# tjysdsg/speech-recognition

Hardware: AMD Instinct MI355X
Metric: frame-state loglik/s + utterances/s Viterbi decode (higher is better)
Workload: dtype f64; 1 GPU; configs[1]: 10-digit HMM, 5 states/digit, 8-mix GMM, 39-dim, 10000 utterances/GPU (999364 frames on rank 0), isolated-word decode; states=50, mixtures=8, dim=39, parallelism=utterance-sharded x1, batches_in_flight=2, process_group=single

## Files before the change

### speech-recognition_amd/csrc/gh_internal.h

```cpp
#pragma once
#include <hip/hip_runtime.h>
#include <stdint.h>
#include <stdarg.h>
#include <stdio.h>
#include <string>
#include <vector>
#include "../../include/gmmhmm.h"

void gh_set_error(const char* fmt, ...);

#define GH_HIP(call)                                                                     \
    do {                                                                                 \
        hipError_t e_ = (call);                                                          \
        if (e_ != hipSuccess) {                                                          \
            gh_set_error("%s:%d %s -> %s", __FILE__, __LINE__, #call, hipGetErrorString(e_)); \
            return (e_ == hipErrorOutOfMemory) ? GH_ERR_NOMEM : GH_ERR_HIP;              \
        }                                                                                \
    } while (0)

#define GH_REQUIRE(cond, ...)                 \
    do {                                      \
        if (!(cond)) {                        \
            gh_set_error(__VA_ARGS__);        \
            return GH_ERR_INVALID;            \
        }                                     \
    } while (0)

#define GH_LEAN_NARROW_ARCS 3

#define GH_LSE_SCALE64 184.66496523378731614
#define GH_LSE_SCALE32 1.4426950408889634074
#define GH_LSE_OFF64 (-1e300)
#define GH_LSE_OFF32 (-1e30f)

struct gh_ctx {
    int device;
    hipStream_t stream;
    int n_cu;
    void* scratch;
    size_t scratch_bytes;
    int* d_flag;
    void* pinned;
    size_t pinned_bytes;
    double* d_fp64_tables;
    int compat;
    int last_fused = 0;
    int last_chunks;
    size_t budget_cache = 0;
    int budget_age = 0;
    void* fit_arena = nullptr;
    size_t fit_arena_bytes = 0;
    void* fit_pin = nullptr;
    void* fit_act = nullptr;
    size_t fit_act_bytes = 0;
};

int gh_scratch(gh_ctx* ctx, size_t bytes, void** out);
size_t gh_scratch_budget(gh_ctx* ctx, bool fresh = false);
int gh_pinned(gh_ctx* ctx, size_t bytes, void** out);

struct gh_gmm {
    gh_ctx* ctx;
    void* d_arena;
    int S, M, D, KP;
    std::vector<double> hA, hB, hC;
    bool host_stale = false;
    double *dA64, *dB64, *dC64;
    float *dA32, *dB32, *dC32;
    float* dCen32;
    double *dMean, *dIvar, *dLogc;
    int* dAnyPos = nullptr;
    int any_pos_host = -1;
    int M_pad, n_tiles;
    double *dApk64, *dCpk64;
    float *dApk32, *dCpk32;
    uint64_t serial = 0;
};
uint64_t gh_next_serial();

#define GH_FBCHAIN_MAX 16
struct gh_fbchain {
    int32_t n, pad;
    int32_t state[GH_FBCHAIN_MAX];
    double c0;
    double self_c[GH_FBCHAIN_MAX], next_c[GH_FBCHAIN_MAX], skip_c[GH_FBCHAIN_MAX];
};

struct gh_batch {
    gh_ctx* ctx;
    gh_dtype dtype;
    int D;
    int64_t N, U;
    void* feats;
    bool owns_feats;
    std::vector<int64_t> offsets;
    int64_t* d_offsets;
    int64_t max_T;
    bool any_T1 = false;
// ... 173 lines not shown
```

### speech-recognition_amd/csrc/gh_loglik_mfma.hip

```cpp
#include <type_traits>
#include "gh_internal.h"
#include "gh_wave.h"

namespace {

typedef double v4d __attribute__((ext_vector_type(4)));
typedef float v4f __attribute__((ext_vector_type(4)));

struct gh_loglik_blk { int64_t n0; int32_t nrows, t0, t1, pad; };

template <typename T> struct Acc;
template <> struct Acc<double> {
    typedef v4d type;
    static __device__ __forceinline__ v4d mfma(double a, double b, v4d c) {
        return __builtin_amdgcn_mfma_f64_16x16x4f64(a, b, c, 0, 0, 0);
    }
};
template <> struct Acc<float> {
    typedef v4f type;
    static __device__ __forceinline__ v4f mfma(float a, float b, v4f c) {
        return __builtin_amdgcn_mfma_f32_16x16x4f32(a, b, c, 0, 0, 0);
    }
};

struct Fp64Tables {
    double exp2[128];
    double inv[128];
    double nlog[128];
};

template <typename T> struct Dom;
template <> struct Dom<double> {
    static constexpr double inv_k = 1.0 / GH_LSE_SCALE64, off = GH_LSE_OFF64, off_test = GH_LSE_OFF64 * 0.1;
};
template <> struct Dom<float> {
    static constexpr float inv_k = (float)(1.0 / GH_LSE_SCALE32), off = GH_LSE_OFF32, off_test = GH_LSE_OFF32 * 0.1f;
};

struct LseK {
    double e3 = 2.6466421444330968834e-08;
    double l4 = -46.166241308446829036, l3 = 61.554988411262438714;
    double l2 = -92.332482616893658071, l1 = 184.66496523378731614;
    __device__ __forceinline__ void pin() {
        asm volatile("" : "+v"(e3), "+v"(l4), "+v"(l3), "+v"(l2), "+v"(l1));
    }
};

__device__ __forceinline__ double logs(double s, const double* __restrict__ tab, const LseK& k) {
    const double* __restrict__ inv = tab + 128;
    const double* __restrict__ nlog = tab + 256;
    const double m = __builtin_amdgcn_frexp_mant(s);
    const int e = __builtin_amdgcn_frexp_exp(s);
    const int j = (__double2hiint(m) >> 13) & 127;
    const double rho = fma(m, inv[j], -1.0);
    double p = fma(rho, 36.932993046757463228, k.l4);
    p = fma(p, rho, k.l3);
    p = fma(p, rho, k.l2);
    p = fma(p, rho, k.l1);
    return fma(p, rho, nlog[j]) + (double)(e << 7);
}
__device__ __forceinline__ float logs(float s, const double*, const LseK&) { return __builtin_amdgcn_logf(s); }

template <int W> __device__ __forceinline__ void swap_rows(unsigned v, unsigned& a, unsigned& b) {
    if (W == 16) {
        auto r = __builtin_amdgcn_permlane16_swap(v, v, false, false);
        a = r[0]; b = r[1];
    } else {
// ... 27 lines not shown
template <typename T> __device__ __forceinline__ T pair_max_split(T v0, T v1) { T a, b; pair_split(v0, v1, a, b); return vmax(a, b); }

template <typename T> __device__ __forceinline__ T nll_of(T mx, T sm, const double* tab, T inf_below, const LseK& k) {
    const T v = (mx + logs(sm, tab, k)) * -Dom<T>::inv_k;
    return (mx < inf_below) ? T(INFINITY) : v;
}

template <typename T, typename V> __device__ __forceinline__ T lane_max(const V& a) { return vmax(vmax(a[0], a[1]), vmax(a[2], a[3])); }
template <typename T, typename V> __device__ __forceinline__ T lane_terms(const V& a, T m, const double* tab, const LseK& k) {
    return (exp2s(a[0] - m, tab, k.e3) + exp2s(a[1] - m, tab, k.e3)) + (exp2s(a[2] - m, tab, k.e3) + exp2s(a[3] - m, tab, k.e3));
}
template <typename T, typename V>
__device__ __forceinline__ void tile_lse(const V& a, int width, T& mx, T& sm, const double* tab, const LseK& k) {
    T m = lane_max<T, V>(a);
    if (width >= 2) m = pair_max<T, 16>(m);
    if (width >= 4) m = pair_max<T, 32>(m);
    T e = lane_terms<T, V>(a, m, tab, k);
    if (width >= 2) e = pair_sum<T, 16>(e);
    if (width >= 4) e = pair_sum<T, 32>(e);
    mx = m;
    sm = e;
}

__device__ __forceinline__ float exp2s_fe(double y) { return __builtin_amdgcn_exp2f((float)y * 0.0078125f); }
template <int W> __device__ __forceinline__ float pair_sum_f(float v) { float a, b; pair_of<W>(v, a, b); return a + b; }
template <typename V>
__device__ __forceinline__ void tile_lse_fe(const V& a, int width, double& mx, float& sm) {
    double m = vmax(vmax(a[0], a[1]), vmax(a[2], a[3]));
    if (width >= 2) m = pair_max<double, 16>(m);
    if (width >= 4) m = pair_max<double, 32>(m);
    float e = (exp2s_fe(a[0] - m) + exp2s_fe(a[1] - m)) + (exp2s_fe(a[2] - m) + exp2s_fe(a[3] - m));
    if (width >= 2) e = pair_sum_f<16>(e);
    if (width >= 4) e = pair_sum_f<32>(e);
    mx = m;
    sm = e;
}
__device__ __forceinline__ double nll_of_fe(double mx, float sm, double inf_below) {
    const double v = (mx + (double)(128.0f * __builtin_amdgcn_logf(sm))) * -Dom<double>::inv_k;
    return (mx < inf_below) ? (double)INFINITY : v;
}

template <typename T> using global_ptr = const T __attribute__((address_space(1)))*;
template <typename T> __device__ __forceinline__ global_ptr<T> uniform_ptr(const T* p) {
    uint32_t lo = (uint32_t)reinterpret_cast<uintptr_t>(p), hi = (uint32_t)(reinterpret_cast<uintptr_t>(p) >> 32);
    asm("" : "+s"(lo), "+s"(hi));
    return (global_ptr<T>)reinterpret_cast<const T*>(((uintptr_t)hi << 32) | lo);
}

template <typename T, typename V, int MP, bool FE = false, bool CHK = true>
__device__ __forceinline__ void tile_epilogue(const V& acc0, const V& acc1, int t, int f, int q, int S, int RS,
                                              int chunk_s0, int tiles_per_state, T* lds, T* dummy,
                                              const double* tab, T (&run_mx)[2], T (&run_sm)[2], T inf_below, const LseK& k) {
    T* orow0 = lds + f * RS - chunk_s0;
    T* orow1 = orow0 + 16 * RS;
    if (MP == 1) {
        const int s = 16 * t + 4 * q;
#pragma unroll
        for (int c = 0; c < 2; ++c) {
            const V& acc = c ? acc1 : acc0;
            T* orow = c ? orow1 : orow0;
#pragma unroll
            for (int r = 0; r < 4; ++r)
                *((!CHK || s + r < S) ? orow + s + r : dummy) = (acc[r] < inf_below) ? T(INFINITY) : acc[r] * -Dom<T>::inv_k;
        }
    } else if (MP == 2) {
        const int s = 8 * t + 2 * q;
#pragma unroll
        for (int c = 0; c < 2; ++c) {
            const V& acc = c ? acc1 : acc0;
            T* orow = c ? orow1 : orow0;
#pragma unroll
            for (int h = 0; h < 2; ++h) {
                const T x0 = acc[2 * h], x1 = acc[2 * h + 1];
                const T m = vmax(x0, x1);
                const T e = exp2s(x0 - m, tab, k.e3) + exp2s(x1 - m, tab, k.e3);
                *((!CHK || s + h < S) ? orow + s + h : dummy) = nll_of<T>(m, e, tab, inf_below, k);
            }
        }
#ifdef GH_MF_NOEPI
    } else if (MP <= 16) {
        const int s = (16 / MP) * t + q / (MP / 4);
        *(((q & (MP / 4 - 1)) == 0 && (!CHK || s < S)) ? orow0 + s : dummy) = -((acc0[0] + acc0[1]) + (acc0[2] + acc0[3]));
        *(((q & (MP / 4 - 1)) == 0 && (!CHK || s < S)) ? orow1 + s : dummy) = -((acc1[0] + acc1[1]) + (acc1[2] + acc1[3]));
#endif
    } else if (FE && MP == 4) {
        if constexpr (FE) {
// ... 27 lines not shown
                const float e = exp2s_fe((d > 0.0) ? -d : d);
                const float rs = (float)run_sm[c];
                run_sm[c] = (double)((d > 0.0) ? fmaf(smf, e, rs) : fmaf(rs, e, smf));
                run_mx[c] = (d > 0.0) ? run_mx[c] : mx;
            }
            const bool odd = q & 1;
            const double v = nll_of_fe(odd ? run_mx[1] : run_mx[0], (float)(odd ? run_sm[1] : run_sm[0]), inf_below);
            *((last && q < 2) ? (odd ? orow1 : orow0) + s : dummy) = v;
#pragma unroll
            for (int c = 0; c < 2; ++c) {
                run_mx[c] = last ? Dom<T>::off : run_mx[c];
                run_sm[c] = last ? T(0) : run_sm[c];
            }
        }
    } else if (MP == 4) {
        T mx, sm;
        const int s = 4 * t + q;
        tile_lse<T, V>(acc0, 1, mx, sm, tab, k);
        *((!CHK || s < S) ? orow0 + s : dummy) = nll_of<T>(mx, sm, tab, inf_below, k);
        tile_lse<T, V>(acc1, 1, mx, sm, tab, k);
        *((!CHK || s < S) ? orow1 + s : dummy) = nll_of<T>(mx, sm, tab, inf_below, k);
    } else if (MP <= 16) {
        constexpr int width = MP / 4;
        T mxs = pair_max_split(lane_max<T, V>(acc0), lane_max<T, V>(acc1));
        if (width >= 4) mxs = pair_max<T, 32>(mxs);
        T mx0, mx1;
        pair_of<16>(mxs, mx0, mx1);
        T sm = pair_sum_split(lane_terms<T, V>(acc0, mx0, tab, k), lane_terms<T, V>(acc1, mx1, tab, k));
        if (width >= 4) sm = pair_sum<T, 32>(sm);
        const bool odd = q & 1;
        const int s = (16 / MP) * t + q / width;
        const T v = nll_of<T>(mxs, sm, tab, inf_below, k);
        *(((q & (width - 1)) < 2 && (!CHK || s < S)) ? (odd ? orow1 : orow0) + s : dummy) = v;
    } else {
        const bool last = (t + 1) % tiles_per_state == 0;
        const int s = t / tiles_per_state;
#pragma unroll
        for (int c = 0; c < 2; ++c) {
            T mx, sm;
            tile_lse<T, V>(c ? acc1 : acc0, 4, mx, sm, tab, k);
            const T d = run_mx[c] - mx;
            const T e = exp2s((d > T(0)) ? -d : d, tab, k.e3);
            run_sm[c] = (d > T(0)) ? fma(sm, e, run_sm[c]) : fma(run_sm[c], e, sm);
            run_mx[c] = (d > T(0)) ? run_mx[c] : mx;
        }
        const bool odd = q & 1;
        const T v = nll_of<T>(odd ? run_mx[1] : run_mx[0], odd ? run_sm[1] : run_sm[0], tab, inf_below, k);
        *((last && q < 2) ? (odd ? orow1 : orow0) + s : dummy) = v;
#pragma unroll
        for (int c = 0; c < 2; ++c) {
            run_mx[c] = last ? Dom<T>::off : run_mx[c];
            run_sm[c] = last ? T(0) : run_sm[c];
        }
    }
}

#ifndef GH_MF_SGB
#define GH_MF_SGB 0
#endif
template <typename T, int KS, int MP, bool MULTI, bool FE = false>
__global__ __launch_bounds__(64, (sizeof(T) == 4 ? 3 : 1)) void loglik_mfma_kernel(const T* __restrict__ X, int64_t N, int D,
                                                         const T* __restrict__ Apk, const T* __restrict__ Cpk,
                                                         int n_tiles, int S, int M_pad, int chunk_tiles,
                                                         const double* __restrict__ tables, int tab_off,
                                                         T* __restrict__ out, int bpw,
                                                         const gh_loglik_blk* __restrict__ blk_tab, int64_t n_blk,
                                                         const T* __restrict__ cen, T inf_below) {
    typedef typename Acc<T>::type V;
#ifndef GH_MF_RING32
#define GH_MF_RING32 2
#endif
#ifndef GH_MF_RING64
#define GH_MF_RING64 1
#endif
    constexpr int R = KS / (sizeof(T) == 4 ? GH_MF_RING32 : GH_MF_RING64);
    extern __shared__ __attribute__((aligned(16))) unsigned char smem_raw[];
    T* lds = reinterpret_cast<T*>(smem_raw);
    const int lane = threadIdx.x;
    const int f = lane & 15, q = lane >> 4;
    const int64_t n_blocks = (N + 31) / 32;
    int64_t n0 = (int64_t)blockIdx.x * (MULTI ? bpw : 1) * 32;
#ifdef GH_MF_TIMING
    long long tk[5], tw[2];
    tk[0] = clock64(); tw[0] = wall_clock64();
#endif
    int nrows = 0;
    const bool subset = MULTI && blk_tab != nullptr;
    const int64_t kb0 = (int64_t)blockIdx.x * (MULTI ? bpw : 1);
    int t_lo = subset ? blk_tab[kb0].t0 : 0, t_hi = n_tiles, nxt_t0 = 0;
    double* tab = reinterpret_cast<double*>(smem_raw + tab_off);
    if (sizeof(T) == 8 && MP != 1) {
        double tr[6];
#pragma unroll
        for (int it = 0; it < 6; ++it) tr[it] = tables[lane + 64 * it];
#pragma unroll
        for (int it = 0; it < 6; ++it) tab[lane + 64 * it] = tr[it];
    }
    auto stage_frames = [&]() {
        const int nelem = nrows * D;
        const T* src = X + n0 * D;
        T xr[KS];
#pragma unroll
        for (int it = 0; it < KS; ++it) {
            const int i = lane + 64 * it;
            xr[it] = (i < nelem) ? src[i] : T(0);
        }
#pragma unroll
        for (int it = 0; it < KS; ++it) {
            const int i = lane + 64 * it;
            if (i < nelem) lds[i] = xr[it];
        }
        __syncthreads();
    };
    constexpr int KQ = KS / 2;
    T b[2][KS];
    T cen_r[KQ];
#pragma unroll
    for (int j = 0; j < KQ; ++j) cen_r[j] = (sizeof(T) == 4 && cen) ? cen[4 * j + q] : T(0);
    auto build_b = [&]() {
#pragma unroll
        for (int c = 0; c < 2; ++c) {
            const int row = 16 * c + f;
#pragma unroll
            for (int j = 0; j < KQ; ++j) {
                const int d = 4 * j + q;
                T v = (row < nrows && d < D) ? lds[row * D + d] : T(0);
                if (sizeof(T) == 4) v = (row < nrows && d < D) ? v - cen_r[j] : T(0);
                b[c][j] = v * v;
                b[c][KQ + j] = v;
            }
        }
        __syncthreads();
    };

    const int tiles_per_state = (MP <= 16) ? 1 : M_pad / 16;
    const int SC = (MP <= 16) ? chunk_tiles * (16 / (MP <= 16 ? MP : 16)) : chunk_tiles / tiles_per_state;
    const int RS = (S <= SC) ? S : SC;
    T* dummy = lds + 32 * RS + lane;
    T run_mx[2] = {Dom<T>::off, Dom<T>::off}, run_sm[2] = {T(0), T(0)};
    LseK lse_k;
    if (sizeof(T) == 8 && !MULTI && !FE && MP != 1) lse_k.pin();
    int chunk_s0 = 0;
    int subset_cnt = 0;

    T ring[R];
#pragma unroll
    for (int j = 0; j < R; ++j) ring[j] = Apk[((int64_t)t_lo * KS + j) * 64 + lane];
    V c_a, c_b, p0, p1;
#pragma unroll
    for (int r = 0; r < 4; ++r) c_a[r] = Cpk[t_lo * 16 + 4 * q + r];

    auto mfma_tile = [&](int t, V& acc0, V& acc1, const V& c_use, V& c_load) {
        const int tn = (!MULTI || t + 1 < t_hi) ? t + 1 : nxt_t0;
        const global_ptr<T> cp = uniform_ptr(Cpk + (unsigned)(tn * 16));
#pragma unroll
        for (int r = 0; r < 4; ++r) c_load[r] = cp[4 * q + r];
        constexpr int WIN = 4096 / (64 * (int)sizeof(T)), NW = (KS + WIN - 1) / WIN;
        global_ptr<T> a_cur[NW], a_nxt[NW];
#pragma unroll
        for (int w = 0; w < NW; ++w) {
            a_cur[w] = uniform_ptr(Apk + (unsigned)(t * (KS * 64) + w * (WIN * 64)));
            a_nxt[w] = uniform_ptr(Apk + (unsigned)(tn * (KS * 64) + w * (WIN * 64)));
        }
#pragma unroll
// ... 46 lines not shown
            const gh_loglik_blk bd = blk_tab[k];
            n0 = bd.n0; nrows = bd.nrows; t_lo = bd.t0; t_hi = bd.t1;
            nxt_t0 = (ib + 1 < nb && k + 1 < n_blk) ? blk_tab[k + 1].t0 : bd.t0;
        } else {
            if (MULTI && n0 >= N) break;
            nrows = (int)((N - n0 < 32) ? (N - n0) : 32);
        }
        if (!(subset && ib > 0 && n0 == staged_n0)) {
#ifdef GH_MF_PRIO
            __builtin_amdgcn_s_setprio(3);
#endif
            stage_frames();
            build_b();
#ifdef GH_MF_PRIO
            __builtin_amdgcn_s_setprio(0);
#endif
            staged_n0 = n0;
        }
        chunk_s0 = (MP <= 16) ? t_lo * (16 / (MP <= 16 ? MP : 16)) : t_lo / tiles_per_state;
        if (subset) {
            const int s_end = (MP <= 16) ? t_hi * (16 / (MP <= 16 ? MP : 16)) : t_hi / tiles_per_state;
            subset_cnt = ((s_end < S) ? s_end : S) - chunk_s0;
        }
#ifdef GH_MF_TIMING
        tk[1] = clock64();
        tk[2] = tk[1];
#endif
        auto epi = [&](const V& e0, const V& e1, int t, auto chk) {
            tile_epilogue<T, V, MP, FE, decltype(chk)::value>(e0, e1, t, f, q, S, RS, chunk_s0, tiles_per_state, lds, dummy, tab, run_mx, run_sm, inf_below, lse_k);
#pragma unroll
            for (int i = 0; i < (GH_MF_SGB ? 2 * KS : 0); ++i) {
                __builtin_amdgcn_sched_group_barrier(0x008, 1, 0);
                __builtin_amdgcn_sched_group_barrier(0x002, sizeof(T) == 8 ? 5 : 3, 0);
            }
            if (!subset && (t + 1) % chunk_tiles == 0 && t + 1 < n_tiles) flush();
        };
        V r0, r1;
        const int tb = MULTI ? t_lo : 0, te = MULTI ? t_hi : n_tiles;
        mfma_tile(tb, p0, p1, c_a, c_b);
        if (sizeof(T) == 8) {
            int t = tb + 1;
            for (; t + 1 < te; t += 2) {
                mfma_tile(t, r0, r1, c_b, c_a);
                epi(p0, p1, t - 1, std::false_type());
                mfma_tile(t + 1, p0, p1, c_a, c_b);
                epi(r0, r1, t, std::false_type());
            }
            if (t < te) {
                mfma_tile(t, r0, r1, c_b, c_a);
                epi(p0, p1, t - 1, std::false_type());
                epi(r0, r1, t, std::true_type());
            } else {
                epi(p0, p1, te - 1, std::true_type());
                if (MULTI) c_a = c_b;
            }
        } else {
            for (int t = tb + 1; t < te; ++t) {
                mfma_tile(t, r0, r1, c_b, c_a);
// ... 54 lines not shown
            runs.push_back({t0, t1});
        }
        std::sort(runs.begin(), runs.end());
        size_t w = 0;
        for (size_t i = 0; i < runs.size(); ++i) {
            if (w > 0 && runs[i].first <= runs[w - 1].second) runs[w - 1].second = std::max(runs[w - 1].second, runs[i].second);
            else runs[w++] = runs[i];
        }
        runs.resize(w);
        for (const auto& tr : runs) {
            const int t0 = tr.first, t1 = tr.second;
            const int span = (M_pad <= 16) ? (t1 - t0) * (16 / M_pad) : (t1 - t0) / (M_pad / 16);
            if (span > SC) return 1;
            max_tiles = std::max(max_tiles, t1 - t0);
        }
        for (int64_t f = b->offsets[u]; f < b->offsets[u + 1]; f += 32)
            for (const auto& tr : runs)
                tabv.push_back(gh_loglik_blk{f, (int32_t)std::min<int64_t>(32, b->offsets[u + 1] - f), tr.first, tr.second, 0});
    }
    *max_tiles_out = max_tiles;
    return GH_OK;
}

template <typename T>
int launch_mfma_t(gh_ctx* ctx, const gh_gmm* g, gh_batch* b, const T* Apk, const T* Cpk, const int32_t* st_lo,
                  const int32_t* st_hi, const T* cen, const int64_t* rng_off, const gh_loglik_plan* plan) {
    const int64_t N = b->N;
    if (N == 0) return GH_OK;
    const int KS = g->KP / 2;
    const int M_pad = g->M_pad, n_tiles = g->n_tiles, S = g->S;
    int chunk_tiles, SC;
    chunk_shape(g, &chunk_tiles, &SC);
    size_t lds = ((size_t)32 * std::max(std::min(SC, S), g->D) + 64) * sizeof(T);
    lds = (lds + 15) & ~size_t(15);
    const int tab_off = (int)lds;
    if (sizeof(T) == 8 && M_pad != 1) lds += 384 * sizeof(double);
    const double* tables = ctx->d_fp64_tables;
    const T inf_below = (ctx->compat & 1) ? (T)(-745.1332191019412 * (sizeof(T) == 8 ? GH_LSE_SCALE64 : GH_LSE_SCALE32)) : Dom<T>::off_test;
    gh_loglik_blk* d_blk = nullptr;
    int64_t n_blk = 0;
    int max_tiles = n_tiles;
    if (plan) {
        d_blk = static_cast<gh_loglik_blk*>(plan->d_blk);
        n_blk = plan->n_blk;
        max_tiles = plan->max_tiles;
        if (n_blk == 0) return GH_OK;
    } else if (st_lo) {
        std::vector<gh_loglik_blk> tabv;
        int rc = build_blk_table(g, b, SC, st_lo, st_hi, rng_off, tabv, &max_tiles);
        if (rc) return rc;
        n_blk = (int64_t)tabv.size();
        if (n_blk == 0) return GH_OK;
        void* base;
        rc = gh_scratch(ctx, tabv.size() * sizeof(gh_loglik_blk), &base);
        if (rc) return rc;
        d_blk = static_cast<gh_loglik_blk*>(base);
        GH_HIP(hipMemcpyAsync(d_blk, tabv.data(), tabv.size() * sizeof(gh_loglik_blk), hipMemcpyHostToDevice, ctx->stream));
        GH_HIP(hipStreamSynchronize(ctx->stream));
    }
    const bool subset = plan || st_lo;
    const int64_t n_blocks = subset ? n_blk : (N + 31) / 32;
    const int per_block = std::max(1, max_tiles * KS * 2);
    int bpw = (int)std::max<int64_t>(1, std::min<int64_t>(8, (512 + per_block - 1) / per_block));
    if (const char* e = getenv("GMMHMM_LOGLIK_BPW")) bpw = std::max(1, std::min(16, atoi(e)));
    if (subset) bpw = std::max(bpw, 2);
    const unsigned grid = (unsigned)((n_blocks + bpw - 1) / bpw);
    const T* X = static_cast<const T*>(b->feats);
    T* out = static_cast<T*>(b->nll);
    const bool fe = sizeof(T) == 8 && (ctx->compat & 2) && M_pad >= 4;
#define GH_MF_LAUNCH(ks, mp)                                                                                             \
    do {                                                                                                                 \
        if (fe && sizeof(T) == 8 && mp >= 4) {                                                                           \
            if (bpw > 1)                                                                                                 \
                hipLaunchKernelGGL((loglik_mfma_kernel<T, ks, mp, true, (sizeof(T) == 8 && mp >= 4)>), dim3(grid), dim3(64), lds, ctx->stream, X, N, g->D, \
                                   Apk, Cpk, n_tiles, S, M_pad, chunk_tiles, tables, tab_off, out, bpw, d_blk, n_blk, cen, inf_below); \
            else                                                                                                         \
                hipLaunchKernelGGL((loglik_mfma_kernel<T, ks, mp, false, (sizeof(T) == 8 && mp >= 4)>), dim3(grid), dim3(64), lds, ctx->stream, X, N, g->D, \
                                   Apk, Cpk, n_tiles, S, M_pad, chunk_tiles, tables, tab_off, out, bpw, d_blk, n_blk, cen, inf_below); \
        } else if (bpw > 1)                                                                                                     \
            hipLaunchKernelGGL((loglik_mfma_kernel<T, ks, mp, true>), dim3(grid), dim3(64), lds, ctx->stream, X, N, g->D, \
                               Apk, Cpk, n_tiles, S, M_pad, chunk_tiles, tables, tab_off, out, bpw, d_blk, n_blk, cen, inf_below); \
        else                                                                                                             \
            hipLaunchKernelGGL((loglik_mfma_kernel<T, ks, mp, false>), dim3(grid), dim3(64), lds, ctx->stream, X, N, g->D, \
                               Apk, Cpk, n_tiles, S, M_pad, chunk_tiles, tables, tab_off, out, bpw, d_blk, n_blk, cen, inf_below); \
    } while (0)
#define GH_MF_CASE(ks)                                   \
    case ks:                                             \
        switch (M_pad) {                                 \
            case 1: GH_MF_LAUNCH(ks, 1); break;          \
            case 2: GH_MF_LAUNCH(ks, 2); break;          \
            case 4: GH_MF_LAUNCH(ks, 4); break;          \
            case 8: GH_MF_LAUNCH(ks, 8); break;          \
            case 16: GH_MF_LAUNCH(ks, 16); break;        \
            default: GH_MF_LAUNCH(ks, 32); break;        \
        }                                                \
        break;
    switch (KS) {
        GH_MF_CASE(2)
        GH_MF_CASE(4)
        GH_MF_CASE(8)
        GH_MF_CASE(12)
        GH_MF_CASE(20)
        GH_MF_CASE(24)
        GH_MF_CASE(32)
        default:
            return 1;
    }
#undef GH_MF_CASE
#undef GH_MF_LAUNCH
    GH_HIP(hipGetLastError());
    return GH_OK;
}

}

int gh_launch_loglik_mfma(gh_ctx* ctx, const gh_gmm* g, gh_batch* b, const int32_t* st_lo, const int32_t* st_hi,
                          const int64_t* rng_off, const gh_loglik_plan* plan) {
    if (!g->dApk64) return 1;
    b->nll_serial = g->serial;
    if (b->dtype == GH_F64) return launch_mfma_t<double>(ctx, g, b, g->dApk64, g->dCpk64, st_lo, st_hi, nullptr, rng_off, plan);
    return launch_mfma_t<float>(ctx, g, b, g->dApk32, g->dCpk32, st_lo, st_hi, g->dCen32, rng_off, plan);
}

int gh_loglik_plan_build(gh_ctx* ctx, const gh_gmm* g, const gh_batch* b, const int32_t* st_lo, const int32_t* st_hi,
                         const int64_t* rng_off, gh_loglik_plan* out, const uint8_t* include) {
    out->d_blk = nullptr; out->n_blk = 0; out->max_tiles = 1;
    if (!g->dApk64) return 1;
    const int KS = g->KP / 2;
    if (KS != 2 && KS != 4 && KS != 8 && KS != 12 && KS != 20 && KS != 24 && KS != 32) return 1;
    int chunk_tiles, SC;
    chunk_shape(g, &chunk_tiles, &SC);
    std::vector<gh_loglik_blk> tabv;
    int rc = build_blk_table(g, b, SC, st_lo, st_hi, rng_off, tabv, &out->max_tiles, include);
    if (rc) return rc;
    out->n_blk = (int64_t)tabv.size();
    if (tabv.empty()) return GH_OK;
    GH_HIP(hipMalloc(&out->d_blk, tabv.size() * sizeof(gh_loglik_blk)));
    GH_HIP(hipMemcpy(out->d_blk, tabv.data(), tabv.size() * sizeof(gh_loglik_blk), hipMemcpyHostToDevice));
    return GH_OK;
}

void gh_loglik_plan_free(gh_loglik_plan* p) {
    if (p && p->d_blk) hipFree(p->d_blk);
    if (p) { p->d_blk = nullptr; p->n_blk = 0; }
// ... 2 lines not shown
```

### speech-recognition_amd/csrc/gh_model.hip

```cpp
#include "gh_internal.h"
#include <atomic>
#include "gh_host.h"

uint64_t gh_next_serial() {
    static std::atomic<uint64_t> counter{0};
    return ++counter;
}

extern "C" int gh_gmm_create(gh_ctx* ctx, int S, int M, int D, const double* mean, const double* var,
                             const double* weight, gh_gmm** out) {
    GH_REQUIRE(ctx && out && mean && var && weight, "gh_gmm_create: NULL argument");
    GH_REQUIRE(S > 0 && M > 0 && D > 0, "gh_gmm_create: S=%d M=%d D=%d must be positive", S, M, D);
    *out = nullptr;
    GH_HIP(hipSetDevice(ctx->device));
    const int G = S * M;
    int KP = (D + 3) & ~3;
    for (const int kp : {4, 8, 16, 24, 40, 48, 64})
        if (KP <= kp) { KP = kp; break; }
    gh_gmm* g = new gh_gmm();
    g->ctx = ctx;
    g->d_arena = nullptr;
    g->S = S; g->M = M; g->D = D; g->KP = KP;
    g->hA.assign((size_t)G * KP, 0.0);
    g->hB.assign((size_t)G * KP, 0.0);
    g->hC.assign(G, 0.0);
    std::vector<double> ivar((size_t)G * D), logc(G);
    const double log2pi = std::log(2.0 * M_PI);
    for (int i = 0; i < G; ++i) {
        double sum_logv = 0, sum_m2 = 0;
// ... 43 lines not shown
    g->M_pad = M_pad;
    g->n_tiles = n_tiles;
    g->dApk64 = nullptr; g->dCpk64 = nullptr; g->dApk32 = nullptr; g->dCpk32 = nullptr; g->dCen32 = nullptr;
    std::vector<double> apk64((size_t)(n_tiles + 2) * KS * 64, 0.0), cpk64((size_t)(n_tiles + 2) * 16, GH_LSE_OFF64);
    std::vector<float> apk32(apk64.size(), 0.f), cpk32(cpk64.size(), GH_LSE_OFF32);
    for (int t = 0; t < n_tiles; ++t)
        for (int j = 0; j < 16; ++j) {
            const int gp = t * 16 + j, s = gp / M_pad, m = gp % M_pad;
            if (s >= S || m >= M) continue;
            const int go = s * M + m;
            const double c = g->hC[go], c32 = hC32[go];
            cpk64[gp] = (c == -INFINITY) ? GH_LSE_OFF64 : std::max(c * GH_LSE_SCALE64, GH_LSE_OFF64);
            cpk32[gp] = (c32 == -INFINITY) ? GH_LSE_OFF32 : (float)std::max(c32 * GH_LSE_SCALE32, (double)GH_LSE_OFF32);
            const int row64 = (j >> 2) + 4 * (j & 3), row32 = j;
            for (int ks = 0; ks < KS; ++ks)
                for (int kq = 0; kq < 4; ++kq) {
                    const int kk = 4 * ks + kq;
                    const double v = kk < KP ? g->hA[(size_t)go * KP + kk] : g->hB[(size_t)go * KP + kk - KP];
                    const double v32 = kk < KP ? v : hB32[(size_t)go * KP + kk - KP];
                    apk64[((size_t)t * KS + ks) * 64 + kq * 16 + row64] = v * GH_LSE_SCALE64;
                    apk32[((size_t)t * KS + ks) * 64 + kq * 16 + row32] = (float)(v32 * GH_LSE_SCALE32);
                }
        }
    std::vector<double> vmean(mean, mean + (size_t)G * D);
    std::vector<int> anypos(1, 0);
    for (int i = 0; i < G; ++i) if (logc[i] > 0) anypos[0] = 1;
    UploadArena ar;
    ar.add(&g->dA64, g->hA); ar.add(&g->dB64, g->hB); ar.add(&g->dC64, g->hC);
    ar.add(&g->dA32, fA); ar.add(&g->dB32, fB); ar.add(&g->dC32, fC); ar.add(&g->dCen32, cen32);
    ar.add(&g->dMean, vmean); ar.add(&g->dIvar, ivar); ar.add(&g->dLogc, logc); ar.add(&g->dAnyPos, anypos);
    g->any_pos_host = anypos[0];
    ar.add(&g->dApk64, apk64); ar.add(&g->dCpk64, cpk64); ar.add(&g->dApk32, apk32); ar.add(&g->dCpk32, cpk32);
    const int rc = ar.commit(&g->d_arena);
    if (rc) {
        gh_gmm_destroy(g);
        return rc;
    }
    g->serial = gh_next_serial();
    *out = g;
    return GH_OK;
}

__global__ __launch_bounds__(1024) void gmm_centre_kernel(const double* __restrict__ mean, int G, int D, int KP, float* __restrict__ cen32,
                                                          int* __restrict__ any_pos) {
    __shared__ double s_acc[16];
    __shared__ int s_cnt[16];
    const int d = blockIdx.x, tid = threadIdx.x, lane = tid & 63, wave = tid >> 6;
    if (d == 0 && tid == 0) *any_pos = 0;
    double acc = 0;
    int cnt = 0;
    if (d < D)
        for (int i = tid; i < G; i += 1024) {
            const double mu = mean[(size_t)i * D + d];
            if (mu - mu == 0.0) { acc += mu; ++cnt; }
        }
#pragma unroll
    for (int o = 32; o >= 1; o >>= 1) { acc += __shfl_xor(acc, o); cnt += __shfl_xor(cnt, o); }
    if (lane == 0) { s_acc[wave] = acc; s_cnt[wave] = cnt; }
    __syncthreads();
    if (tid == 0) {
        double a = 0;
        int n = 0;
        for (int w = 0; w < 16; ++w) { a += s_acc[w]; n += s_cnt[w]; }
        float c = n ? (float)(a / n) : 0.f;
        if (!(c - c == 0.f)) c = 0.f;
        cen32[d] = c;
    }
}

struct gmm_dev_view {
    int* any_pos;
    int S, M, D, KP, M_pad, n_tiles;
    double *A64, *B64, *C64, *Mean, *Ivar, *Logc, *Apk64, *Cpk64;
    float *A32, *B32, *C32, *Apk32, *Cpk32;
    const float* cen32;
};

__global__ void gmm_pack_plain_kernel(gmm_dev_view v, const double* __restrict__ mean, const double* __restrict__ var,
                                      const double* __restrict__ weight, int* __restrict__ flag) {
    const int i = blockIdx.x * blockDim.x + threadIdx.x;
    const int G = v.S * v.M;
    if (i >= G) return;
    const int D = v.D, KP = v.KP;
    const double log2pi = 1.8378770664093454836;
    double sum_logv = 0, sum_m2 = 0, sum_m2c = 0;
    for (int d = 0; d < D; ++d) {
        const double vv = var[(size_t)i * D + d], mu = mean[(size_t)i * D + d];
        if (vv == 0) atomicOr(flag, 16);
        const double iv = 1.0 / vv;
        const double muc = mu - (double)v.cen32[d];
        v.Mean[(size_t)i * D + d] = mu;
        v.Ivar[(size_t)i * D + d] = iv;
        v.A64[(size_t)i * KP + d] = -0.5 * iv;
        v.B64[(size_t)i * KP + d] = mu * iv;
        v.A32[(size_t)i * KP + d] = (float)(-0.5 * iv);
        v.B32[(size_t)i * KP + d] = (float)(muc * iv);
        sum_logv += log(vv);
        sum_m2 += mu * mu * iv;
        sum_m2c += muc * muc * iv;
    }
    const double logc = log(weight[i]) - 0.5 * (D * log2pi + sum_logv);
    v.Logc[i] = logc;
    if (logc > 0) atomicOr(v.any_pos, 1);
    const double c = logc - 0.5 * sum_m2, c32 = logc - 0.5 * sum_m2c;
    v.C64[i] = c;
    v.C32[i] = (float)c32;
    const int s = i / v.M, m = i - s * v.M;
    const int gp = s * v.M_pad + m;
    v.Cpk64[gp] = (c == -INFINITY) ? GH_LSE_OFF64 : fmax(c * GH_LSE_SCALE64, GH_LSE_OFF64) + (c != c ? c : 0.0);
    v.Cpk32[gp] = (c32 == -INFINITY) ? GH_LSE_OFF32 : (float)(fmax(c32 * GH_LSE_SCALE32, (double)GH_LSE_OFF32) + (c32 != c32 ? c32 : 0.0));
}

__global__ void gmm_pack_operands_kernel(gmm_dev_view v) {
    const int64_t idx = (int64_t)blockIdx.x * blockDim.x + threadIdx.x;
    const int K2 = 2 * v.KP;
    const int64_t total = (int64_t)v.n_tiles * 16 * K2;
    if (idx >= total) return;
    const int gp = (int)(idx / K2), kk = (int)(idx - (int64_t)gp * K2);
    const int s = gp / v.M_pad, m = gp - s * v.M_pad;
    if (s >= v.S || m >= v.M) return;
    const int go = s * v.M + m;
    const int t = gp >> 4, j = gp & 15;
    const int KS = v.KP / 2, ks = kk >> 2, kq = kk & 3;
    const int row64 = (j >> 2) + 4 * (j & 3), row32 = j;
    const double a64 = kk < v.KP ? v.A64[(size_t)go * v.KP + kk] : v.B64[(size_t)go * v.KP + kk - v.KP];
    double a32 = a64;
    if (kk >= v.KP) {
        const int d = kk - v.KP;
        a32 = d < v.D ? (v.Mean[(size_t)go * v.D + d] - (double)v.cen32[d]) * v.Ivar[(size_t)go * v.D + d] : 0.0;
    }
    v.Apk64[((size_t)t * KS + ks) * 64 + kq * 16 + row64] = a64 * GH_LSE_SCALE64;
    v.Apk32[((size_t)t * KS + ks) * 64 + kq * 16 + row32] = (float)(a32 * GH_LSE_SCALE32);
}

int gh_gmm_update_dev(gh_ctx* ctx, gh_gmm* g, const double* d_mean, const double* d_var, const double* d_weight, int* d_flag) {
    const int G = g->S * g->M;
    hipStream_t st = ctx->stream;
    gmm_dev_view v;
    v.S = g->S; v.M = g->M; v.D = g->D; v.KP = g->KP; v.M_pad = g->M_pad; v.n_tiles = g->n_tiles;
    v.A64 = g->dA64; v.B64 = g->dB64; v.C64 = g->dC64; v.Mean = g->dMean; v.Ivar = g->dIvar; v.Logc = g->dLogc;
    v.Apk64 = g->dApk64; v.Cpk64 = g->dCpk64; v.A32 = g->dA32; v.B32 = g->dB32; v.C32 = g->dC32;
    v.Apk32 = g->dApk32; v.Cpk32 = g->dCpk32; v.cen32 = g->dCen32; v.any_pos = g->dAnyPos;
    g->any_pos_host = -1;
    hipLaunchKernelGGL(gmm_centre_kernel, dim3(g->KP), dim3(1024), 0, st, d_mean, G, g->D, g->KP, g->dCen32, g->dAnyPos);
    hipLaunchKernelGGL(gmm_pack_plain_kernel, dim3((G + 63) / 64), dim3(64), 0, st, v, d_mean, d_var, d_weight, d_flag);
    const int64_t total = (int64_t)g->n_tiles * 16 * 2 * g->KP;
    hipLaunchKernelGGL(gmm_pack_operands_kernel, dim3((unsigned)((total + 255) / 256)), dim3(256), 0, st, v);
    GH_HIP(hipGetLastError());
    g->host_stale = true;
    g->serial = gh_next_serial();
    return GH_OK;
}

extern "C" int gh_gmm_update(gh_ctx* ctx, gh_gmm* g, const double* mean, const double* var, const double* weight) {
    GH_REQUIRE(ctx && g && mean && var && weight, "gh_gmm_update: NULL argument");
    GH_HIP(hipSetDevice(ctx->device));
    const size_t G = (size_t)g->S * g->M, nd = G * g->D;
    for (size_t i = 0; i < nd; ++i)
        GH_REQUIRE(var[i] != 0, "gh_gmm_update: var[%zu,%zu,%zu]=0 (singular covariance)", i / g->D / g->M, i / g->D % g->M, i % g->D);
    void* base;
    int rc = gh_scratch(ctx, (2 * nd + G) * 8, &base);
    if (rc) return rc;
    double* d = static_cast<double*>(base);
    GH_HIP(hipMemcpyAsync(d, mean, nd * 8, hipMemcpyHostToDevice, ctx->stream));
    GH_HIP(hipMemcpyAsync(d + nd, var, nd * 8, hipMemcpyHostToDevice, ctx->stream));
    GH_HIP(hipMemcpyAsync(d + 2 * nd, weight, G * 8, hipMemcpyHostToDevice, ctx->stream));
    rc = gh_gmm_update_dev(ctx, g, d, d + nd, d + 2 * nd, ctx->d_flag);
    if (rc) return rc;
// ... 448 lines not shown
```

Baseline: 43.21 billion frame-state loglik/s.

## Use pack-time per-state max bound to skip max-shift in fp64 log-sum-exp

At pack time, each state's mixture constants are shifted by the largest per-state log-weight, and a lower threshold for the resulting sum is precomputed. The fp64 MFMA epilogue then sums exp2 terms directly, without the runtime max reduction and subtraction. A wave-wide ballot falls back to the original max-shifted log-sum-exp only when some sum falls below the threshold. This removes the cross-lane max reductions and subtractions from the hot epilogue, at the cost of extra LDS staging of per-state bounds, more template variants, and a rare cold path.

New measurement: 43.75 billion frame-state loglik/s (median of 6 runs). +1.2%, better.

```diff
diff --git a/speech-recognition_amd/csrc/gh_internal.h b/speech-recognition_amd/csrc/gh_internal.h
--- a/speech-recognition_amd/csrc/gh_internal.h
+++ b/speech-recognition_amd/csrc/gh_internal.h
@@ -32,6 +32,19 @@
 #define GH_LSE_SCALE32 1.4426950408889634074
 #define GH_LSE_OFF64 (-1e300)
 #define GH_LSE_OFF32 (-1e30f)
+#define GH_LSE_COMPAT_BELOW64 (-745.1332191019412 * GH_LSE_SCALE64)
+#define GH_LSE_BOUND_THR 0x1p-900
+struct gh_lse_state { double k_mh, thr; };
+__host__ __device__ inline gh_lse_state gh_lse_state_of(double mh, bool any_on, int M_pad) {
+    gh_lse_state e;
+    if (!any_on) { e.k_mh = 0.0; e.thr = INFINITY; return e; }
+    e.k_mh = mh * GH_LSE_SCALE64;
+    const double ex = (GH_LSE_COMPAT_BELOW64 - e.k_mh) * (1.0 / 128.0);
+    const double t = (ex > 1000.0) ? (double)INFINITY : ((ex < -1060.0) ? 0.0 : ldexp(exp2(ex - floor(ex)), (int)floor(ex)) * (2.0 * M_pad));
+    e.thr = (t > GH_LSE_BOUND_THR) ? t : GH_LSE_BOUND_THR;
+    return e;
+}
+static inline int gh_lse_states_padded(int M_pad, int n_tiles) { return n_tiles * (16 / M_pad); }
 
 struct gh_ctx {
     int device;
@@ -74,6 +87,8 @@
     int M_pad, n_tiles;
     double *dApk64, *dCpk64;
     float *dApk32, *dCpk32;
+    double* dCpkRel64 = nullptr;
+    gh_lse_state* dLseState64 = nullptr;
     uint64_t serial = 0;
 };
 uint64_t gh_next_serial();
diff --git a/speech-recognition_amd/csrc/gh_loglik_mfma.hip b/speech-recognition_amd/csrc/gh_loglik_mfma.hip
--- a/speech-recognition_amd/csrc/gh_loglik_mfma.hip
+++ b/speech-recognition_amd/csrc/gh_loglik_mfma.hip
@@ -43,6 +43,9 @@
     double l2 = -92.332482616893658071, l1 = 184.66496523378731614;
     __device__ __forceinline__ void pin() {
         asm volatile("" : "+v"(e3), "+v"(l4), "+v"(l3), "+v"(l2), "+v"(l1));
+    }
+    __device__ __forceinline__ void pin_bnd() {
+        asm volatile("" : "+v"(e3), "+v"(l4), "+s"(l3), "+s"(l2), "+s"(l1));
     }
 };
 
@@ -116,6 +119,29 @@
     sm = e;
 }
 
+template <typename T, typename V, int W>
+__device__ __forceinline__ void wide_lse(const V& acc0, const V& acc1, T& mxs, T& sm, const double* tab, const LseK& k) {
+    mxs = pair_max_split(lane_max<T, V>(acc0), lane_max<T, V>(acc1));
+    if (W >= 4) mxs = pair_max<T, 32>(mxs);
+    T mx0, mx1;
+    pair_of<16>(mxs, mx0, mx1);
+    sm = pair_sum_split(lane_terms<T, V>(acc0, mx0, tab, k), lane_terms<T, V>(acc1, mx1, tab, k));
+    if (W >= 4) sm = pair_sum<T, 32>(sm);
+}
+
+template <typename T, typename V> __device__ __forceinline__ T lane_terms0(const V& a, const double* tab, const LseK& k) {
+    return (exp2s(a[0], tab, k.e3) + exp2s(a[1], tab, k.e3)) + (exp2s(a[2], tab, k.e3) + exp2s(a[3], tab, k.e3));
+}
+template <typename T> __device__ __forceinline__ T nll_bnd(T k_mh, T sm, const double* tab, const LseK& k) {
+    return (k_mh + logs(sm, tab, k)) * -Dom<T>::inv_k;
+}
+template <typename T> __device__ __forceinline__ T nll_cold(T mx, T sm, T k_mh, const double* tab, T inf_below, const LseK& k) {
+    const T v = ((mx + logs(sm, tab, k)) + k_mh) * -Dom<T>::inv_k;
+    return (mx + k_mh < inf_below) ? T(INFINITY) : v;
+}
+__device__ __forceinline__ bool wave_any(bool p) { return __builtin_amdgcn_ballot_w64(p) != 0; }
+__device__ __forceinline__ void cold_block() { asm volatile("; log-sum-exp redo (max-shifted)" ::: "memory"); }
+
 __device__ __forceinline__ float exp2s_fe(double y) { return __builtin_amdgcn_exp2f((float)y * 0.0078125f); }
 template <int W> __device__ __forceinline__ float pair_sum_f(float v) { float a, b; pair_of<W>(v, a, b); return a + b; }
 template <typename V>
@@ -141,10 +167,12 @@
     return (global_ptr<T>)reinterpret_cast<const T*>(((uintptr_t)hi << 32) | lo);
 }
 
-template <typename T, typename V, int MP, bool FE = false, bool CHK = true>
+template <typename T, typename V, int MP, bool FE = false, bool CHK = true, bool BND = false>
 __device__ __forceinline__ void tile_epilogue(const V& acc0, const V& acc1, int t, int f, int q, int S, int RS,
                                               int chunk_s0, int tiles_per_state, T* lds, T* dummy,
-                                              const double* tab, T (&run_mx)[2], T (&run_sm)[2], T inf_below, const LseK& k) {
+                                              const double* tab, T (&run_mx)[2], T (&run_sm)[2], T inf_below, const LseK& k,
+                                              const double* st_tab) {
+    static_assert(!BND || (MP >= 2 && MP <= 16), "the bound form covers one tile per state");
     T* orow0 = lds + f * RS - chunk_s0;
     T* orow1 = orow0 + 16 * RS;
     if (MP == 1) {
@@ -156,6 +184,76 @@
 #pragma unroll
             for (int r = 0; r < 4; ++r)
                 *((!CHK || s + r < S) ? orow + s + r : dummy) = (acc[r] < inf_below) ? T(INFINITY) : acc[r] * -Dom<T>::inv_k;
+        }
+    } else if (BND) {
+        if constexpr (BND) {
+            const double* st = st_tab - 2 * chunk_s0;
+            if (MP == 2) {
+                const int s = 8 * t + 2 * q;
+                const T km[2] = {st[2 * s], st[2 * s + 2]}, th[2] = {st[2 * s + 1], st[2 * s + 3]};
+                T v[2][2];
+                bool redo[2][2], cold = false;
+#pragma unroll
+                for (int c = 0; c < 2; ++c) {
+                    const V& acc = c ? acc1 : acc0;
+#pragma unroll
+                    for (int h = 0; h < 2; ++h) {
+                        const T e = exp2s(acc[2 * h], tab, k.e3) + exp2s(acc[2 * h + 1], tab, k.e3);
+                        redo[c][h] = e < th[h];
+                        cold |= redo[c][h];
+                        v[c][h] = nll_bnd<T>(km[h], e, tab, k);
+                    }
+                }
+                if (__builtin_expect(wave_any(cold), 0)) {
+                    cold_block();
+#pragma unroll
+                    for (int c = 0; c < 2; ++c) {
+                        const V& acc = c ? acc1 : acc0;
+#pragma unroll
+                        for (int h = 0; h < 2; ++h) {
+                            const T x0 = acc[2 * h], x1 = acc[2 * h + 1];
+                            const T m = vmax(x0, x1);
+                            const T e = exp2s(x0 - m, tab, k.e3) + exp2s(x1 - m, tab, k.e3);
+                            v[c][h] = redo[c][h] ? nll_cold<T>(m, e, km[h], tab, inf_below, k) : v[c][h];
+                        }
+                    }
+                }
+#pragma unroll
+                for (int c = 0; c < 2; ++c)
+#pragma unroll
+                    for (int h = 0; h < 2; ++h) *((!CHK || s + h < S) ? (c ? orow1 : orow0) + s + h : dummy) = v[c][h];
+            } else if (MP == 4) {
+                const int s = 4 * t + q;
+                const T km = st[2 * s], th = st[2 * s + 1];
+                const T e0 = lane_terms0<T, V>(acc0, tab, k), e1 = lane_terms0<T, V>(acc1, tab, k);
+                T v0 = nll_bnd<T>(km, e0, tab, k), v1 = nll_bnd<T>(km, e1, tab, k);
+                if (__builtin_expect(wave_any((e0 < th) | (e1 < th)), 0)) {
+                    cold_block();
+                    T mx, sm;
+                    tile_lse<T, V>(acc0, 1, mx, sm, tab, k);
+                    v0 = (e0 < th) ? nll_cold<T>(mx, sm, km, tab, inf_below, k) : v0;
+                    tile_lse<T, V>(acc1, 1, mx, sm, tab, k);
+                    v1 = (e1 < th) ? nll_cold<T>(mx, sm, km, tab, inf_below, k) : v1;
+                }
+                *((!CHK || s < S) ? orow0 + s : dummy) = v0;
+                *((!CHK || s < S) ? orow1 + s : dummy) = v1;
+            } else {
+                constexpr int width = MP / 4;
+                T sm = pair_sum_split(lane_terms0<T, V>(acc0, tab, k), lane_terms0<T, V>(acc1, tab, k));
+                if (width >= 4) sm = pair_sum<T, 32>(sm);
+                const bool odd = q & 1;
+                const int s = (16 / MP) * t + q / width;
+                const T km = st[2 * s], th = st[2 * s + 1];
+                const bool redo = wave_any(sm < th);
+                T v = nll_bnd<T>(km, sm, tab, k);
+                if (__builtin_expect(redo, 0)) {
+                    cold_block();
+                    T mxs, smc;
+                    wide_lse<T, V, width>(acc0, acc1, mxs, smc, tab, k);
+                    v = (sm < th) ? nll_cold<T>(mxs, smc, km, tab, inf_below, k) : v;
+                }
+                *(((q & (width - 1)) < 2 && (!CHK || s < S)) ? (odd ? orow1 : orow0) + s : dummy) = v;
+            }
         }
     } else if (MP == 2) {
         const int s = 8 * t + 2 * q;
@@ -229,12 +327,8 @@
         *((!CHK || s < S) ? orow1 + s : dummy) = nll_of<T>(mx, sm, tab, inf_below, k);
     } else if (MP <= 16) {
         constexpr int width = MP / 4;
-        T mxs = pair_max_split(lane_max<T, V>(acc0), lane_max<T, V>(acc1));
-        if (width >= 4) mxs = pair_max<T, 32>(mxs);
-        T mx0, mx1;
-        pair_of<16>(mxs, mx0, mx1);
-        T sm = pair_sum_split(lane_terms<T, V>(acc0, mx0, tab, k), lane_terms<T, V>(acc1, mx1, tab, k));
-        if (width >= 4) sm = pair_sum<T, 32>(sm);
+        T mxs, sm;
+        wide_lse<T, V, width>(acc0, acc1, mxs, sm, tab, k);
         const bool odd = q & 1;
         const int s = (16 / MP) * t + q / width;
         const T v = nll_of<T>(mxs, sm, tab, inf_below, k);
@@ -265,14 +359,16 @@
 #ifndef GH_MF_SGB
 #define GH_MF_SGB 0
 #endif
-template <typename T, int KS, int MP, bool MULTI, bool FE = false>
+template <typename T, int KS, int MP, bool MULTI, bool FE = false, bool BND = false>
 __global__ __launch_bounds__(64, (sizeof(T) == 4 ? 3 : 1)) void loglik_mfma_kernel(const T* __restrict__ X, int64_t N, int D,
                                                          const T* __restrict__ Apk, const T* __restrict__ Cpk,
                                                          int n_tiles, int S, int M_pad, int chunk_tiles,
                                                          const double* __restrict__ tables, int tab_off,
                                                          T* __restrict__ out, int bpw,
                                                          const gh_loglik_blk* __restrict__ blk_tab, int64_t n_blk,
-                                                         const T* __restrict__ cen, T inf_below) {
+                                                         const T* __restrict__ cen, T inf_below,
+                                                         const gh_lse_state* __restrict__ st_glob, int st_off) {
+    static_assert(!BND || (sizeof(T) == 8 && !FE && MP >= 2 && MP <= 16), "the pack-time bound is for the default fp64 log-sum-exp, one tile per state");
     typedef typename Acc<T>::type V;
 #ifndef GH_MF_RING32
 #define GH_MF_RING32 2
@@ -296,6 +392,28 @@
     const int64_t kb0 = (int64_t)blockIdx.x * (MULTI ? bpw : 1);
     int t_lo = subset ? blk_tab[kb0].t0 : 0, t_hi = n_tiles, nxt_t0 = 0;
     double* tab = reinterpret_cast<double*>(smem_raw + tab_off);
+    double* st_tab = reinterpret_cast<double*>(smem_raw + st_off);
+    const int tiles_per_state = (MP <= 16) ? 1 : M_pad / 16;
+    const int SC = (MP <= 16) ? chunk_tiles * (16 / (MP <= 16 ? MP : 16)) : chunk_tiles / tiles_per_state;
+    const int st_n = n_tiles * (16 / (MP <= 16 ? MP : 16));
+    int st_s0 = -1;
+    auto stage_states = [&](int s0) {
+        if constexpr (BND) {
+            const int cnt = (st_n - s0 < SC) ? st_n - s0 : SC;
+            const bool compat = inf_below > Dom<T>::off_test;
+            gh_lse_state e[2];
+#pragma unroll
+            for (int it = 0; it < 2; ++it) e[it] = (lane + 64 * it < cnt) ? st_glob[s0 + lane + 64 * it] : gh_lse_state{0.0, 0.0};
+#pragma unroll
+            for (int it = 0; it < 2; ++it)
+                if (lane + 64 * it < cnt) {
+                    st_tab[2 * (lane + 64 * it)] = e[it].k_mh;
+                    st_tab[2 * (lane + 64 * it) + 1] = compat ? e[it].thr : ((e[it].thr == 0.0) ? 0.0 : GH_LSE_BOUND_THR);
+                }
+            st_s0 = s0;
+        }
+    };
+    if (BND) stage_states(t_lo * (16 / (MP <= 16 ? MP : 16)));
     if (sizeof(T) == 8 && MP != 1) {
         double tr[6];
 #pragma unroll
@@ -340,13 +458,11 @@
         __syncthreads();
     };
 
-    const int tiles_per_state = (MP <= 16) ? 1 : M_pad / 16;
-    const int SC = (MP <= 16) ? chunk_tiles * (16 / (MP <= 16 ? MP : 16)) : chunk_tiles / tiles_per_state;
     const int RS = (S <= SC) ? S : SC;
     T* dummy = lds + 32 * RS + lane;
     T run_mx[2] = {Dom<T>::off, Dom<T>::off}, run_sm[2] = {T(0), T(0)};
     LseK lse_k;
-    if (sizeof(T) == 8 && !MULTI && !FE && MP != 1) lse_k.pin();
+    if (sizeof(T) == 8 && !MULTI && !FE && MP != 1) { if (BND) lse_k.pin_bnd(); else lse_k.pin(); }
     int chunk_s0 = 0;
     int subset_cnt = 0;
 
@@ -439,18 +555,22 @@
             const int s_end = (MP <= 16) ? t_hi * (16 / (MP <= 16 ? MP : 16)) : t_hi / tiles_per_state;
             subset_cnt = ((s_end < S) ? s_end : S) - chunk_s0;
         }
+        if (BND && st_s0 != chunk_s0) { stage_states(chunk_s0); __syncthreads(); }
 #ifdef GH_MF_TIMING
         tk[1] = clock64();
         tk[2] = tk[1];
 #endif
         auto epi = [&](const V& e0, const V& e1, int t, auto chk) {
-            tile_epilogue<T, V, MP, FE, decltype(chk)::value>(e0, e1, t, f, q, S, RS, chunk_s0, tiles_per_state, lds, dummy, tab, run_mx, run_sm, inf_below, lse_k);
+            tile_epilogue<T, V, MP, FE, decltype(chk)::value, BND>(e0, e1, t, f, q, S, RS, chunk_s0, tiles_per_state, lds, dummy, tab, run_mx, run_sm, inf_below, lse_k, st_tab);
 #pragma unroll
             for (int i = 0; i < (GH_MF_SGB ? 2 * KS : 0); ++i) {
                 __builtin_amdgcn_sched_group_barrier(0x008, 1, 0);
                 __builtin_amdgcn_sched_group_barrier(0x002, sizeof(T) == 8 ? 5 : 3, 0);
             }
-            if (!subset && (t + 1) % chunk_tiles == 0 && t + 1 < n_tiles) flush();
+            if (!subset && (t + 1) % chunk_tiles == 0 && t + 1 < n_tiles) {
+                flush();
+                if (BND) { stage_states(chunk_s0); __syncthreads(); }
+            }
         };
         V r0, r1;
         const int tb = MULTI ? t_lo : 0, te = MULTI ? t_hi : n_tiles;
@@ -551,8 +671,13 @@
     return GH_OK;
 }
 
+static bool lse_bound_enabled() {
+    const char* e = getenv("GMMHMM_LSE_BOUND");
+    return !(e && e[0] == '0' && e[1] == 0);
+}
+
 template <typename T>
-int launch_mfma_t(gh_ctx* ctx, const gh_gmm* g, gh_batch* b, const T* Apk, const T* Cpk, const int32_t* st_lo,
+int launch_mfma_t(gh_ctx* ctx, const gh_gmm* g, gh_batch* b, const T* Apk, const T* Cpk, const T* CpkRel, const int32_t* st_lo,
                   const int32_t* st_hi, const T* cen, const int64_t* rng_off, const gh_loglik_plan* plan) {
     const int64_t N = b->N;
     if (N == 0) return GH_OK;
@@ -564,6 +689,9 @@
     lds = (lds + 15) & ~size_t(15);
     const int tab_off = (int)lds;
     if (sizeof(T) == 8 && M_pad != 1) lds += 384 * sizeof(double);
+    const bool bnd = sizeof(T) == 8 && M_pad != 1 && M_pad <= 16 && !((ctx->compat & 2) && M_pad >= 4) && CpkRel && g->dLseState64 && lse_bound_enabled();
+    const int st_off = (int)lds;
+    if (bnd) lds += (size_t)std::min(SC, gh_lse_states_padded(M_pad, n_tiles)) * sizeof(gh_lse_state);
     const double* tables = ctx->d_fp64_tables;
     const T inf_below = (ctx->compat & 1) ? (T)(-745.1332191019412 * (sizeof(T) == 8 ? GH_LSE_SCALE64 : GH_LSE_SCALE32)) : Dom<T>::off_test;
     gh_loglik_blk* d_blk = nullptr;
@@ -597,21 +725,23 @@
     const T* X = static_cast<const T*>(b->feats);
     T* out = static_cast<T*>(b->nll);
     const bool fe = sizeof(T) == 8 && (ctx->compat & 2) && M_pad >= 4;
+#define GH_MF_LAUNCH1(ks, mp, multi, fe_, bnd_)                                                                          \
+    hipLaunchKernelGGL((loglik_mfma_kernel<T, ks, mp, multi, fe_, bnd_>), dim3(grid), dim3(64), lds, ctx->stream, X, N, g->D, \
+                       Apk, bnd ? CpkRel : Cpk, n_tiles, S, M_pad, chunk_tiles, tables, tab_off, out, bpw, d_blk, n_blk, cen, \
+                       inf_below, g->dLseState64, st_off)
 #define GH_MF_LAUNCH(ks, mp)                                                                                             \
     do {                                                                                                                 \
-        if (fe && sizeof(T) == 8 && mp >= 4) {                                                                           \
-            if (bpw > 1)                                                                                                 \
-                hipLaunchKernelGGL((loglik_mfma_kernel<T, ks, mp, true, (sizeof(T) == 8 && mp >= 4)>), dim3(grid), dim3(64), lds, ctx->stream, X, N, g->D, \
-                                   Apk, Cpk, n_tiles, S, M_pad, chunk_tiles, tables, tab_off, out, bpw, d_blk, n_blk, cen, inf_below); \
-            else                                                                                                         \
-                hipLaunchKernelGGL((loglik_mfma_kernel<T, ks, mp, false, (sizeof(T) == 8 && mp >= 4)>), dim3(grid), dim3(64), lds, ctx->stream, X, N, g->D, \
-                                   Apk, Cpk, n_tiles, S, M_pad, chunk_tiles, tables, tab_off, out, bpw, d_blk, n_blk, cen, inf_below); \
-        } else if (bpw > 1)                                                                                                     \
-            hipLaunchKernelGGL((loglik_mfma_kernel<T, ks, mp, true>), dim3(grid), dim3(64), lds, ctx->stream, X, N, g->D, \
-                               Apk, Cpk, n_tiles, S, M_pad, chunk_tiles, tables, tab_off, out, bpw, d_blk, n_blk, cen, inf_below); \
+        constexpr bool f64 = sizeof(T) == 8;                                                                             \
+        if (fe && f64 && mp >= 4) {                                                                                      \
+            if (bpw > 1) GH_MF_LAUNCH1(ks, mp, true, (f64 && mp >= 4), false);                                           \
+            else GH_MF_LAUNCH1(ks, mp, false, (f64 && mp >= 4), false);                                                  \
+        } else if (bnd && f64 && mp != 1 && mp <= 16) {                                                                  \
+            if (bpw > 1) GH_MF_LAUNCH1(ks, mp, true, false, (f64 && mp != 1 && mp <= 16));                               \
+            else GH_MF_LAUNCH1(ks, mp, false, false, (f64 && mp != 1 && mp <= 16));                                      \
+        } else if (bpw > 1)                                                                                              \
+            GH_MF_LAUNCH1(ks, mp, true, false, false);                                                                   \
         else                                                                                                             \
-            hipLaunchKernelGGL((loglik_mfma_kernel<T, ks, mp, false>), dim3(grid), dim3(64), lds, ctx->stream, X, N, g->D, \
-                               Apk, Cpk, n_tiles, S, M_pad, chunk_tiles, tables, tab_off, out, bpw, d_blk, n_blk, cen, inf_below); \
+            GH_MF_LAUNCH1(ks, mp, false, false, false);                                                                  \
     } while (0)
 #define GH_MF_CASE(ks)                                   \
     case ks:                                             \
@@ -637,6 +767,7 @@
     }
 #undef GH_MF_CASE
 #undef GH_MF_LAUNCH
+#undef GH_MF_LAUNCH1
     GH_HIP(hipGetLastError());
     return GH_OK;
 }
@@ -647,8 +778,8 @@
                           const int64_t* rng_off, const gh_loglik_plan* plan) {
     if (!g->dApk64) return 1;
     b->nll_serial = g->serial;
-    if (b->dtype == GH_F64) return launch_mfma_t<double>(ctx, g, b, g->dApk64, g->dCpk64, st_lo, st_hi, nullptr, rng_off, plan);
-    return launch_mfma_t<float>(ctx, g, b, g->dApk32, g->dCpk32, st_lo, st_hi, g->dCen32, rng_off, plan);
+    if (b->dtype == GH_F64) return launch_mfma_t<double>(ctx, g, b, g->dApk64, g->dCpk64, g->dCpkRel64, st_lo, st_hi, nullptr, rng_off, plan);
+    return launch_mfma_t<float>(ctx, g, b, g->dApk32, g->dCpk32, (const float*)nullptr, st_lo, st_hi, g->dCen32, rng_off, plan);
 }
 
 int gh_loglik_plan_build(gh_ctx* ctx, const gh_gmm* g, const gh_batch* b, const int32_t* st_lo, const int32_t* st_hi,
diff --git a/speech-recognition_amd/csrc/gh_model.hip b/speech-recognition_amd/csrc/gh_model.hip
--- a/speech-recognition_amd/csrc/gh_model.hip
+++ b/speech-recognition_amd/csrc/gh_model.hip
@@ -5,6 +5,21 @@
 uint64_t gh_next_serial() {
     static std::atomic<uint64_t> counter{0};
     return ++counter;
+}
+
+__host__ __device__ inline void gh_pack_lse_state(const double* c, const double* logc, int M, int M_pad, double* rel, gh_lse_state* st) {
+    double mh = -INFINITY;
+    bool any_on = false, all_nan = (M == M_pad);
+    for (int m = 0; m < M; ++m) {
+        if (c[m] - c[m] == 0.0 && logc[m] - logc[m] == 0.0 && c[m] * GH_LSE_SCALE64 > GH_LSE_OFF64) { any_on = true; mh = (logc[m] > mh) ? logc[m] : mh; }
+        all_nan = all_nan && c[m] != c[m];
+    }
+    *st = gh_lse_state_of(mh, any_on, M_pad);
+    for (int m = 0; m < M; ++m) {
+        const double r = (c[m] - mh) * GH_LSE_SCALE64;
+        if (!any_on) rel[m] = all_nan ? c[m] : GH_LSE_OFF64;
+        else rel[m] = (c[m] == -INFINITY) ? GH_LSE_OFF64 : ((r > GH_LSE_OFF64) ? r : GH_LSE_OFF64) + (c[m] != c[m] ? c[m] : 0.0);
+    }
 }
 
 extern "C" int gh_gmm_create(gh_ctx* ctx, int S, int M, int D, const double* mean, const double* var,
@@ -94,6 +109,10 @@
                     apk32[((size_t)t * KS + ks) * 64 + kq * 16 + row32] = (float)(v32 * GH_LSE_SCALE32);
                 }
         }
+    const bool lse_bound = M_pad >= 2 && M_pad <= 16;
+    std::vector<double> cpkrel64(lse_bound ? cpk64.size() : 0, GH_LSE_OFF64);
+    std::vector<gh_lse_state> lse_state(lse_bound ? gh_lse_states_padded(M_pad, n_tiles) : 0, gh_lse_state{0.0, 0.0});
+    for (int s = 0; lse_bound && s < S; ++s) gh_pack_lse_state(&g->hC[(size_t)s * M], &logc[(size_t)s * M], M, M_pad, &cpkrel64[(size_t)s * M_pad], &lse_state[s]);
     std::vector<double> vmean(mean, mean + (size_t)G * D);
     std::vector<int> anypos(1, 0);
     for (int i = 0; i < G; ++i) if (logc[i] > 0) anypos[0] = 1;
@@ -103,6 +122,7 @@
     ar.add(&g->dMean, vmean); ar.add(&g->dIvar, ivar); ar.add(&g->dLogc, logc); ar.add(&g->dAnyPos, anypos);
     g->any_pos_host = anypos[0];
     ar.add(&g->dApk64, apk64); ar.add(&g->dCpk64, cpk64); ar.add(&g->dApk32, apk32); ar.add(&g->dCpk32, cpk32);
+    ar.add(&g->dCpkRel64, cpkrel64); ar.add(&g->dLseState64, lse_state);
     const int rc = ar.commit(&g->d_arena);
     if (rc) {
         gh_gmm_destroy(g);
@@ -143,7 +163,8 @@
 struct gmm_dev_view {
     int* any_pos;
     int S, M, D, KP, M_pad, n_tiles;
-    double *A64, *B64, *C64, *Mean, *Ivar, *Logc, *Apk64, *Cpk64;
+    double *A64, *B64, *C64, *Mean, *Ivar, *Logc, *Apk64, *Cpk64, *CpkRel64;
+    gh_lse_state* LseState64;
     float *A32, *B32, *C32, *Apk32, *Cpk32;
     const float* cen32;
 };
@@ -183,6 +204,12 @@
     v.Cpk32[gp] = (c32 == -INFINITY) ? GH_LSE_OFF32 : (float)(fmax(c32 * GH_LSE_SCALE32, (double)GH_LSE_OFF32) + (c32 != c32 ? c32 : 0.0));
 }
 
+__global__ void gmm_pack_lse_kernel(gmm_dev_view v) {
+    const int s = blockIdx.x * blockDim.x + threadIdx.x;
+    if (s >= v.S) return;
+    gh_pack_lse_state(v.C64 + (size_t)s * v.M, v.Logc + (size_t)s * v.M, v.M, v.M_pad, v.CpkRel64 + (size_t)s * v.M_pad, v.LseState64 + s);
+}
+
 __global__ void gmm_pack_operands_kernel(gmm_dev_view v) {
     const int64_t idx = (int64_t)blockIdx.x * blockDim.x + threadIdx.x;
     const int K2 = 2 * v.KP;
@@ -213,9 +240,11 @@
     v.A64 = g->dA64; v.B64 = g->dB64; v.C64 = g->dC64; v.Mean = g->dMean; v.Ivar = g->dIvar; v.Logc = g->dLogc;
     v.Apk64 = g->dApk64; v.Cpk64 = g->dCpk64; v.A32 = g->dA32; v.B32 = g->dB32; v.C32 = g->dC32;
     v.Apk32 = g->dApk32; v.Cpk32 = g->dCpk32; v.cen32 = g->dCen32; v.any_pos = g->dAnyPos;
+    v.CpkRel64 = g->dCpkRel64; v.LseState64 = g->dLseState64;
     g->any_pos_host = -1;
     hipLaunchKernelGGL(gmm_centre_kernel, dim3(g->KP), dim3(1024), 0, st, d_mean, G, g->D, g->KP, g->dCen32, g->dAnyPos);
     hipLaunchKernelGGL(gmm_pack_plain_kernel, dim3((G + 63) / 64), dim3(64), 0, st, v, d_mean, d_var, d_weight, d_flag);
+    if (g->dCpkRel64) hipLaunchKernelGGL(gmm_pack_lse_kernel, dim3((g->S + 63) / 64), dim3(64), 0, st, v);
     const int64_t total = (int64_t)g->n_tiles * 16 * 2 * g->KP;
     hipLaunchKernelGGL(gmm_pack_operands_kernel, dim3((unsigned)((total + 255) / 256)), dim3(256), 0, st, v);
     GH_HIP(hipGetLastError());
```
